# frankaging/Multimodal-Transformer

Measured on AMD Instinct MI355X. Metric: windows/sec fwd+bwd, higher is better.
Workload: dtype bf16; 1 GPU; SFT encoder stack T=500 d_model=128 heads=8 N=6 d_ff=128, 32 sequences/GPU; fwd + MSE loss + bwd (input, weight, LayerNorm grads); global_batch=32, seq_len=500, d_model=128, heads=8, layers=6, d_ff=128, parallelism=dp1, dropout=train mode, p=0.10 at the reference's four encoder sites, in-kernel generator, lengths=full

## Files before the change

include/mmt_hip.h:

```cpp
#ifndef MMT_HIP_H
#define MMT_HIP_H
#include <stddef.h>
#include <stdint.h>

#ifdef __cplusplus
extern "C" {
#endif

#define MMT_OK 0
#define MMT_EINVAL 1
#define MMT_EUNSUPPORTED 2
#define MMT_EWORKSPACE 3
#define MMT_EHIP 4

typedef void* mmt_stream_t;

int mmt_abi_version(void);
const char* mmt_last_error(void);

int mmt_profile_enable(int on);
int mmt_profile_reset(void);
int mmt_profile_num_sites(void);
const char* mmt_profile_site_name(int site);
int mmt_profile_collect(float* total_ms, int* launches);
// ... 266 lines not shown
                            void* workspace, size_t workspace_bytes, int N, int W, int D, int F, int K, mmt_stream_t stream);

size_t mmt_mse_sum_scratch_doubles(size_t n);
int mmt_mse_sum_forward(const float* pred, const float* target, float inv_denom, float* loss, float* dpred, double* scratch,
                        size_t n, mmt_stream_t stream);

int mmt_adam_step(float* const* params, const float* const* grads, float* const* exp_avg, float* const* exp_avg_sq,
                  const size_t* counts, int nchunks, float lr, float beta1, float beta2, float eps, float weight_decay,
                  int step, mmt_stream_t stream);

int mmt_ccc_forward(const float* pred, const float* target, const int32_t* lengths, double* ccc, int B, int T, mmt_stream_t stream);

int mmt_debug_dropout_mask(float p, uint64_t seed, uint32_t stream_id, uint64_t n, uint32_t attn_Tp, uint8_t* keep,
                           float* host_scale_out, mmt_stream_t stream);

int mmt_debug_poison_lds(uint32_t pattern, void* sink4, mmt_stream_t stream);

#ifdef __cplusplus
}
#endif
#endif
```

multimodal_transformer_amd/_lib.py:

```python
import ctypes
import os
import threading

import torch

_HERE = os.path.dirname(os.path.abspath(__file__))
LIB_PATH = os.environ.get("MMT_LIB_PATH") or os.path.join(_HERE, "libmmt_hip.so")

_c = ctypes
_P, _F, _I, _SZ, _U64 = _c.c_void_p, _c.c_float, _c.c_int, _c.c_size_t, _c.c_uint64

SIGNATURES = {
    "mmt_abi_version": (_I, []),
    "mmt_last_error": (_c.c_char_p, []),
    "mmt_profile_enable": (_I, [_I]),
    "mmt_profile_reset": (_I, []),
    "mmt_profile_num_sites": (_I, []),
    "mmt_profile_site_name": (_c.c_char_p, [_I]),
    "mmt_profile_collect": (_I, [_P, _P]),
    "mmt_encoder_param_count": (_SZ, [_I, _I, _I]),
    "mmt_encoder_workspace_bytes": (_SZ, [_I] * 6),
    "mmt_encoder_workspace_bytes_eval": (_SZ, [_I] * 6),
    "mmt_encoder_forward": (_I, [_P, _P, _P, _P, _P, _SZ] + [_I] * 6 + [_F, _F, _U64, _P]),
    "mmt_encoder_backward": (_I, [_P, _P, _P, _P, _P, _P, _P, _SZ] + [_I] * 6 + [_F, _F, _U64, _P]),
# ... 80 lines not shown
    "mmt_mfn_mem_scan_forward": (_I, [_P] * 9 + [_SZ] + [_I] * 4 + [_F, _U64, _P]),
    "mmt_mfn_mem_scan_forward_devseed": (_I, [_P] * 9 + [_SZ] + [_I] * 4 + [_F, _P, _P]),
    "mmt_mfn_mem_scan_backward": (_I, [_P] * 11 + [_SZ] + [_I] * 4 + [_F, _P]),
    "mmt_convpool_workspace_bytes": (_SZ, [_I] * 4),
    "mmt_convpool_forward": (_I, [_P] * 6 + [_SZ] + [_I] * 4 + [_P]),
    "mmt_convpool_backward": (_I, [_P] * 6 + [_SZ] + [_I] * 4 + [_P]),
    "mmt_convpool_k_workspace_bytes": (_SZ, [_I] * 5),
    "mmt_convpool_k_forward": (_I, [_P] * 6 + [_SZ] + [_I] * 5 + [_P]),
    "mmt_convpool_k_backward": (_I, [_P] * 6 + [_SZ] + [_I] * 5 + [_P]),
    "mmt_mse_sum_scratch_doubles": (_SZ, [_SZ]),
    "mmt_mse_sum_forward": (_I, [_P, _P, _F, _P, _P, _P, _SZ, _P]),
    "mmt_adam_step": (_I, [_P, _P, _P, _P, _P, _I, _F, _F, _F, _F, _F, _I, _P]),
    "mmt_ccc_forward": (_I, [_P, _P, _P, _P, _I, _I, _P]),
    "mmt_debug_dropout_mask": (_I, [_F, _U64, _c.c_uint32, _U64, _c.c_uint32, _P, _P, _P]),
    "mmt_debug_poison_lds": (_I, [_c.c_uint32, _P, _P]),
}


class CopySeg(ctypes.Structure):
    _fields_ = [("src", _P), ("src2", _P), ("dst", _P), ("rowscale", _P), ("rows", _I), ("cols", _I), ("src_ld", _I), ("src2_ld", _I),
                ("dst_ld", _I), ("perm", _I), ("pB", _I), ("pT", _I), ("accumulate", _I)]


_lib = None
_lock = threading.Lock()


def load():
    global _lib
    if _lib is not None:
# ... 290 lines not shown
```

multimodal_transformer_amd/csrc/api.hip:

```cpp
#include <hip/hip_runtime.h>
#include <stdarg.h>
#include <stdio.h>
#include <string.h>
#include <math.h>
#include <stdlib.h>
#include <initializer_list>
#include <mutex>
#include <type_traits>
#include <unordered_set>

#include "../../include/mmt_hip.h"
#include "common.h"
#include "attn_mask.h"
#include "rowgemm.h"
#include "attn.h"
#include "attn_bwd_pair.h"
#include "attn_probs.h"
#ifdef MMT_ABLATIONS
#include "attn_bwd_pair_diag.h"
#include "attn_fwd_diag.h"
#endif
#include "misc_kernels.h"
#include "scan_common.h"
#include "scan.h"
// ... 184 lines not shown
    D.nsplit = (D.MP + D.mchunk - 1) / D.mchunk;
    return MMT_OK;
}

static int check_drop(float dropout_p, const EncDims& D) {
    if (!(dropout_p >= 0.f && dropout_p < 1.f)) return fail(MMT_EINVAL, "dropout_p %g not in [0,1)", dropout_p);
    if (dropout_p > 0.f && D.Tp > 4096) return fail(MMT_EUNSUPPORTED, "train-mode dropout supports T <= 4096 (got %d)", D.T);
    return MMT_OK;
}

static bool use_fused_bwd(const EncDims& D) {
    static const bool allowed = getenv("MMT_NO_FUSED_ATTN_BWD") == nullptr;
    return allowed && attn_bwd_fused_ok(D.L.DKP, D.nt);
}

struct LayerWs {
    float *xout, *x1, *stats1, *stats2, *lse;
    bf16 *xn1, *xn2, *QR, *KR, *VR, *ctx, *hid;
    bf16 *dx2, *dh, *dx1, *dqkv;
    float *lnpart1, *lnpart2;
    uint16_t *maskQ, *maskK;
};
struct EncWs {
    uint64_t* seedword;
    bf16* wprep; float* bprep; float* statsf;
    LayerWs lw[MAX_LAYERS];
    float *dxa, *dxb, *delta, *lnpartf;
    bf16 *dOR;
    float *sWqkv, *sbqkv, *sWo, *sbo, *sW1, *sb1, *sW2, *sb2;
    size_t slab_stride;
// ... 116 lines not shown
static bool prep_shape_at(int shape) { return tail_fold_on() && shape == 128; }
static RowGemmParams rg_zero() { RowGemmParams p; memset(&p, 0, sizeof(p)); p.mask_scale = 1.0f; return p; }

static DropCfg no_drop() { return make_drop(0.f, 0, 0); }
#define MMT_ATTN_DROP_BITS 12
static DropCfg stream_drop(float p, uint64_t seed, uint32_t stream, bool devseed, int bits = 16, uint32_t first = 0) {
    DropCfg c = make_drop(p, seed, stream, bits);
    if (devseed) { c.s0 = stream - first; c.s1 = 0; }
    return c;
}
static int launch_seed_advance(uint64_t* state, uint64_t* block, uint32_t first, int n, hipStream_t st) {
    if (n + 1 > MMT_SEED_BLOCK_WORDS) return fail(MMT_EUNSUPPORTED, "%d dropout streams do not fit the seed block", n);
    return launch("seed_advance_kernel", seed_advance_kernel, dim3(1), dim3(128), 0, st, state, block, first, n);
}

static int fill_mask_gen(MaskGenParams& P, uint16_t* mq, uint16_t* mk, const EncDims& D, int nlayers, float p, uint64_t seed,
                         const uint64_t* seedword = nullptr) {
    if (nlayers > 16) return fail(MMT_EUNSUPPORTED, "mask generator: %d layers > 16", nlayers);
    memset(&P, 0, sizeof(P));
    P.lq = mq; P.lk = mk; P.nbh = D.B * D.h; P.nt = D.nt; P.nlayers = nlayers;
    P.layer_words = attn_mask_layer_words(P.nbh, P.nt);
    P.seedword = seedword;
    for (int l = 0; l < nlayers; ++l) { const DropCfg c = stream_drop(p, seed, 4 * l + 0, seedword != nullptr, MMT_ATTN_DROP_BITS); P.thr16 = c.thr16; P.s0[l] = c.s0; P.s1[l] = c.s1; }
    return MMT_OK;
}
static int launch_mask_gen(uint16_t* mq, uint16_t* mk, const EncDims& D, int nlayers, float p, uint64_t seed, hipStream_t st) {
    MaskGenParams P;
    int rc;
    if ((rc = fill_mask_gen(P, mq, mk, D, nlayers, p, seed))) return rc;
    const size_t blocks = (size_t)P.nbh * P.nt * P.nt;
    ProfScope prof(S_MASK_GEN, st);
    return launch("attn_mask_gen_kernel", attn_mask_gen_kernel, dim3((unsigned)((blocks + 255) / 256), nlayers), dim3(256), 0, st, P);
}

class AttnSel {
    AttnSel(AttnMode m, const int32_t* kl, int sp = 0) : mode(m), key_lengths(kl), span(sp) {}
public:
    AttnMode mode; const int32_t* key_lengths; int span;
    static AttnSel plain() { return AttnSel(ATTN_PLAIN, nullptr); }
    static AttnSel causal() { return AttnSel(ATTN_CAUSAL, nullptr); }
    static AttnSel band(int span) { return AttnSel(ATTN_BAND, nullptr, span); }
    static AttnSel keys(const int32_t* key_lengths) { return AttnSel(ATTN_KEYS, key_lengths); }
};
template <typename KP, typename KK, typename KB, typename... A>
static int launch_attn_form(const AttnSel& sel, const char* plain_name, KP* plain, const char* keys_name, KK* keys, const char* causal_name, KP* causal,
                            const char* band_name, KB* band, dim3 grid, hipStream_t st, const A&... args) {
    if (sel.mode == ATTN_KEYS) return launch(keys_name, keys, grid, dim3(MMT_THREADS), 0, st, args..., sel.key_lengths);
    if (sel.mode == ATTN_BAND) return launch(band_name, band, grid, dim3(MMT_THREADS), 0, st, args..., sel.span);
    const bool c = sel.mode == ATTN_CAUSAL;
    return launch(c ? causal_name : plain_name, c ? causal : plain, grid, dim3(MMT_THREADS), 0, st, args...);
}

static int launch_attn_fwd(int DKP, const bf16* QR, const bf16* KR, const bf16* VR, bf16* ctx, float* lse,
                           const EncDims& D, hipStream_t st, const AttnSel& sel, DropCfg drop = no_drop(), const uint16_t* maskQ = nullptr) {
    dim3 grid(attn_grid((D.nt + 3) / 4, D.B * D.h));
    if (drop.thr16 && !maskQ) return fail(MMT_EINVAL, "attention dropout without a mask buffer");
    ProfScope prof(S_ATTN_FWD, st);
#ifdef MMT_ABLATIONS
    static const bool stamp_fwd = getenv("MMT_ABL") && atoi(getenv("MMT_ABL")) == 6;
    if (stamp_fwd && sel.mode == ATTN_PLAIN && DKP == 16 && drop.thr16)
        return launch("attn_fwd_stamped_kernel", attn_fwd_stamped_kernel<16, true>, grid, dim3(MMT_THREADS), 0, st, QR, KR, VR, ctx, lse,
                      D.h, D.T, D.nt, D.B * D.h, D.L.HDP, maskQ, drop.scale, 0);
#endif
    return with_dkp(DKP, drop.thr16 != 0, [&](auto dkp, auto dr) {
        int rc = MMT_OK;
        for (int fb = 0; fb < (CT(dkp) + 31) / 32 && !rc; ++fb)
            rc = launch_attn_form(sel, "attn_fwd_kernel", attn_fwd_kernel<CT(dkp), CT(dr)>, "attn_fwd_keys_kernel", attn_fwd_keys_kernel<CT(dkp), CT(dr)>,
                                  "attn_fwd_causal_kernel", attn_fwd_causal_kernel<CT(dkp), CT(dr)>,
                                  "attn_fwd_band_kernel", attn_fwd_band_kernel<CT(dkp), CT(dr)>, grid, st,
                                  QR, KR, VR, ctx, lse, D.h, D.T, D.nt, D.B * D.h, D.L.HDP, maskQ, drop.scale, fb);
        return rc;
    });
}

static int launch_attn_bwd(int DKP, const bf16* QR, const bf16* KR, const bf16* VR,
                           const bf16* dOR, const float* lse, const float* delta, const float* rowmask,
                           bf16* dqkv, const EncDims& D, hipStream_t st, const AttnSel& sel, DropCfg drop = no_drop(),
                           const uint16_t* maskQ = nullptr, const uint16_t* maskK = nullptr) {
// ... 82 lines not shown
    if (!pointers_ok || !workspace) return fail(MMT_EINVAL, "null pointer argument");
    if ((rc = check_drop(dropout_p, C.D))) return rc;
    carve_encoder(C.W, C.D, workspace, dropout_p > 0.f);
    if ((rc = check_workspace(workspace_bytes, C.W.bytes))) return rc;
    C.st = static_cast<hipStream_t>(stream);
    C.dropout_p = dropout_p; C.seed = seed;
    C.devseed = devseed && dropout_p > 0.f;
    C.seedword = C.devseed ? C.W.seedword : nullptr;
    return MMT_OK;
}
static MaskRide layer_mask_ride(const MaskGenParams& MG, const EncWs& W, int layer, int waves, int chain_wgs) {
    MaskRide ride; memset(&ride, 0, sizeof(ride));
    ride.chain_wgs = chain_wgs;
    if (!waves) return ride;
    MaskGenLayer& g = ride.g;
    g.lq = W.lw[layer].maskQ; g.lk = W.lw[layer].maskK; g.nbh = MG.nbh; g.nt = MG.nt;
    g.thr16 = MG.thr16; g.s0 = MG.s0[layer]; g.s1 = MG.s1[layer]; g.seedword = MG.seedword;
    const size_t blocks = (size_t)g.nbh * g.nt * g.nt, per_wg = (size_t)64 * waves;
    ride.gen_waves = waves; ride.gen_wgs = (int)((blocks + per_wg - 1) / per_wg);
    return ride;
}

static int encoder_forward_impl(const float* x, const float* mask, const float* params, float* y,
                                void* workspace, size_t workspace_bytes,
                                int B, int T, int d, int h, int f, int n_layers, float eps,
                                float dropout_p, uint64_t seed, uint64_t* seed_state, mmt_stream_t stream, const AttnSel& sel) {
    EncCall C;
    C.sel = sel;
    int rc = encoder_begin(C, x && mask && params && y, workspace, workspace_bytes, B, T, d, h, f, n_layers, dropout_p, seed, seed_state != nullptr, stream);
    if (rc) return rc;
    ALIGNED16("mmt_encoder_forward", PA(x), PA(params), PA(y));
    const EncDims& D = C.D; const EncWs& W = C.W; const LayerLayout& L = D.L;
    hipStream_t st = C.st;
    const bool devseed = C.devseed;
    const uint64_t* seedword = C.seedword;

    const int shape = chain_shape(d, f, h, L);
    static const bool fuse_next_qkv = getenv("MMT_NO_CHAIN4") == nullptr;
    const int ride_waves = (dropout_p > 0.f && fuse_next_qkv)
        ? mask_ride_waves(shape, layer_geom(CHAIN_FWD, L).lds) : 0;
    const int head_waves = (dropout_p > 0.f && fuse_next_qkv && D.N > 0 && (D.N == 1 || ride_waves))
        ? mask_ride_waves(shape, layer_geom(STAGE_LN1_QKV, L).lds, MMT_HEAD_RIDE_WAVES) : 0;
    const int nstreams = 4 * D.N + 4;
    if (devseed && !head_waves && (rc = launch_seed_advance(seed_state, W.seedword, 0, nstreams, st))) return rc;
    MaskGenParams MG;
    if (D.N > 0 && dropout_p > 0.f && (rc = fill_mask_gen(MG, W.lw[0].maskQ, W.lw[0].maskK, D, D.N, dropout_p, seed, seedword))) return rc;
    if (D.N > 0 && dropout_p > 0.f && !head_waves) {
        MaskGenParams P = MG;
        if (ride_waves) P.nlayers = 1;
        const size_t blocks = (size_t)P.nbh * P.nt * P.nt;
        const int gen_blocks = (int)((blocks + 255) / 256), prep_blocks = std::min(grid_for(L.pstride() + L.qstride()), 64);
        ProfScope prof(S_MASK_GEN, st);
        LAUNCH(encoder_prep_maskgen_kernel, dim3((unsigned)(gen_blocks + prep_blocks), D.N), dim3(256), 0, st,
                           params, W.wprep, W.bprep, L, gen_blocks, P);
    } else if (D.N > 0) {
        if (devseed && nstreams + 1 > MMT_SEED_BLOCK_WORDS) return fail(MMT_EUNSUPPORTED, "%d dropout streams do not fit the seed block", nstreams);
        ProfScope prof(S_PREP, st);
        if (prep_shape_at(shape)) {
            const int prep_blocks = PrepShape<128>::blocks();
            if (devseed) LAUNCH(encoder_prep_shape_seed_kernel<128>, dim3(prep_blocks + 1, D.N), dim3(256), 0, st,
                               params, W.wprep, W.bprep, L, seed_state, W.seedword, nstreams);
// ... 440 lines not shown
}

static int sdpa_forward_impl(const float* q, const float* k, const float* v, const float* mask, float* ctx,
                             void* workspace, size_t workspace_bytes, int B, int T, int d, int h,
                             float dropout_p, uint64_t seed, mmt_stream_t stream, const AttnSel& sel) {
    SdpaCall C;
    int rc = sdpa_begin(C, q && k && v && ctx, workspace, workspace_bytes, B, T, d, h, dropout_p, stream);
    if (rc) return rc;
    const EncDims& D = C.D; const SdpaWs& W = C.W; const LayerLayout& L = D.L;
    hipStream_t st = C.st;
    const int g = grid_for((size_t)D.M * h);
    const float qs = LOG2E / sqrtf((float)L.dk);
    LAUNCH(pack_frag_kernel, dim3(g), dim3(256), 0, st, q, W.QR, mask, qs, 1, nullptr, 0, nullptr, D.M, T, D.Tp, h, L.dk, L.DKP, d);
    LAUNCH(pack_frag_kernel, dim3(g), dim3(256), 0, st, k, W.KR, nullptr, 1.f, 0, nullptr, 0, nullptr, D.M, T, D.Tp, h, L.dk, L.DKP, d);
    LAUNCH(pack_frag_kernel, dim3(g), dim3(256), 0, st, v, W.VR, nullptr, 1.f, 0, nullptr, 0, nullptr, D.M, T, D.Tp, h, L.dk, L.DKP, d);
    if (dropout_p > 0.f && (rc = launch_mask_gen(W.maskQ, W.maskK, D, 1, dropout_p, seed, st))) return rc;
    if ((rc = launch_attn_fwd(L.DKP, W.QR, W.KR, W.VR, W.ctx, W.lse, D, st, sel, make_drop(dropout_p, seed, 0, MMT_ATTN_DROP_BITS), W.maskQ))) return rc;
    LAUNCH(unpad_heads_kernel, dim3(grid_for((size_t)D.M * d)), dim3(256), 0, st, W.ctx, L.HDP, 0, ctx, D.M, h, L.dk, L.DKP, d);
    return MMT_OK;
}
extern "C" int mmt_sdpa_forward(const float* q, const float* k, const float* v, const float* mask, float* ctx,
                                void* workspace, size_t workspace_bytes, int B, int T, int d, int h,
                                float dropout_p, uint64_t seed, mmt_stream_t stream) {
    return sdpa_forward_impl(q, k, v, mask, ctx, workspace, workspace_bytes, B, T, d, h, dropout_p, seed, stream, AttnSel::plain());
}
extern "C" int mmt_sdpa_forward_keys(const float* q, const float* k, const float* v, const float* mask, float* ctx,
                                     void* workspace, size_t workspace_bytes, int B, int T, int d, int h,
                                     float dropout_p, uint64_t seed, mmt_stream_t stream, const int32_t* key_lengths) {
    if (!key_lengths) return fail(MMT_EINVAL, "null key_lengths");
    return sdpa_forward_impl(q, k, v, mask, ctx, workspace, workspace_bytes, B, T, d, h, dropout_p, seed, stream, AttnSel::keys(key_lengths));
}
// ... 1215 lines not shown

extern "C" int mmt_ccc_forward(const float* pred, const float* target, const int32_t* lengths, double* ccc, int B, int T, mmt_stream_t stream) {
    if (!pred || !target || !lengths || !ccc) return fail(MMT_EINVAL, "null pointer argument");
    if (B <= 0 || T <= 0) return fail(MMT_EINVAL, "bad shape B=%d T=%d", B, T);
    LAUNCH(ccc_kernel, dim3(B), dim3(256), 0, static_cast<hipStream_t>(stream), pred, target, lengths, ccc, T);
    return MMT_OK;
}

extern "C" int mmt_debug_poison_lds(uint32_t pattern, void* sink4, mmt_stream_t stream) {
    if (!sink4) return fail(MMT_EINVAL, "null pointer argument");
    LAUNCH(poison_lds_kernel, dim3(2048), dim3(1024), 160 * 1024, static_cast<hipStream_t>(stream), pattern, 160 * 256, static_cast<uint32_t*>(sink4));
    LAUNCH(poison_vgpr_kernel, dim3(8192), dim3(256), 0, static_cast<hipStream_t>(stream), pattern, static_cast<uint32_t*>(sink4));
    return MMT_OK;
}

extern "C" int mmt_debug_dropout_mask(float p, uint64_t seed, uint32_t stream_id, uint64_t n, uint32_t attn_Tp, uint8_t* keep,
                                      float* scale_out, mmt_stream_t stream) {
    if (!keep) return fail(MMT_EINVAL, "null pointer argument");
    const DropCfg c = make_drop(p, seed, stream_id, attn_Tp ? MMT_ATTN_DROP_BITS : 16);
    if (scale_out) *scale_out = c.scale;
    if (attn_Tp) {
        if (attn_Tp % 32 || n % ((uint64_t)attn_Tp * attn_Tp)) return fail(MMT_EINVAL, "attention mask: n must be a multiple of Tp*Tp, Tp of 32");
        const int nt = (int)(attn_Tp / 32), nbh = (int)(n / ((uint64_t)attn_Tp * attn_Tp));
        const size_t blocks = (size_t)nbh * nt * nt;
        LAUNCH(attn_mask_expand_kernel, dim3((unsigned)((blocks + 63) / 64)), dim3(64), 0, static_cast<hipStream_t>(stream), c, nbh, nt, keep);
        return MMT_OK;
    }
    LAUNCH(dropout_mask_kernel, dim3(grid_for(n)), dim3(256), 0, static_cast<hipStream_t>(stream), c, n, keep);
    return MMT_OK;
}
// ... 1 lines not shown
```

multimodal_transformer_amd/csrc/attn.h:

```cpp
#pragma once
#include <type_traits>
#include "common.h"
#include "attn_mask.h"

template <int NSEG, int MAXL = 3>
struct TileStager {
    const bf16* src[MAXL]; int stride[MAXL]; bool on[MAXL]; int dst[MAXL];
    bf16x8 reg[MAXL];
    __device__ __forceinline__ void init(const bf16* const* base, const int* pieces, const int* strides, const int* lds0, const int* pad, int tid) {
#pragma unroll
        for (int l = 0; l < MAXL; ++l) {
            const int p = tid + MMT_THREADS * l;
            int acc = 0; on[l] = false; src[l] = base[0]; stride[l] = 0; dst[l] = 0;
#pragma unroll
            for (int sg = 0; sg < NSEG; ++sg) {
                if (!on[l] && p >= acc && p < acc + pieces[sg]) {
                    on[l] = true; src[l] = base[sg] + (size_t)(p - acc) * 8; stride[l] = strides[sg];
                    dst[l] = (lds0[sg] + (p - acc) + ((p - acc) >> 5) * pad[sg]) * 8;
                }
                acc += pieces[sg];
            }
        }
    }
    __device__ __forceinline__ void load(int tile) {
// ... 44 lines not shown
    const int L = blockIdx.x, grp = L / (8 * nx), rem = L - grp * 8 * nx;
    AttnBlock a;
    a.bx = rem >> 3;
    a.bh = grp * 8 + (rem & 7);
    a.valid = a.bh < nbh;
    return a;
}
__host__ inline int attn_grid(int nx, int nbh) { return nx * 8 * ((nbh + 7) / 8); }
__device__ __forceinline__ AttnBlock attn_block_causal(int nx, int nbh) {
    AttnBlock a = attn_block(nx, nbh);
    const int grp = blockIdx.x / (8 * nx);
    a.bx = (a.bx + ((grp * nx) >> 5)) % nx;
    return a;
}

template <int DKP, bool DROP, int MODE>
__device__ __forceinline__ void attn_fwd_body(
        const bf16* __restrict__ Qr, const bf16* __restrict__ Kr, const bf16* __restrict__ Vr,
        bf16* __restrict__ ctx, float* __restrict__ lse,
        int h, int T, int nt, int nbh, int ldc, const uint16_t* __restrict__ maskQ, float drop_scale, int fb,
        const int* __restrict__ key_lengths, int span) {
    constexpr bool KEYS = MODE == ATTN_KEYS, CAUSAL = MODE == ATTN_CAUSAL, BAND = MODE == ATTN_BAND;
    constexpr int KS = DKP / 16;
    constexpr int DKB = DKP < 32 ? DKP : 32;
    constexpr bool ONES = (DKP == 16) && !DROP;
    constexpr int PK = DKP * 4, PV = DKB * 4, PVL = (DKB / 8) * MMT_TR_OCT;
    __shared__ __attribute__((aligned(16))) bf16 stage[2][(PK + PVL) * 8];
    __shared__ __attribute__((aligned(16))) bf16 zeros[256];
    const int lane = threadIdx.x & 63, wave = __builtin_amdgcn_readfirstlane(threadIdx.x >> 6);
    const int r = lane & 31, hh = lane >> 5;
    const AttnBlock ab = CAUSAL ? attn_block_causal((nt + 3) >> 2, nbh) : attn_block((nt + 3) >> 2, nbh);
    if (!ab.valid) return;
    const int qt = ab.bx * 4 + wave;
    const bool live = qt < nt;
    const int qtc = live ? qt : nt - 1;
    const int bh = ab.bh, b = bh / h, head = bh - b * h;
    const int Tp = nt * 32;
    const int Tk = KEYS ? attn_key_len(key_lengths, b, T) : T;
    const int nk = KEYS ? (Tk + 31) >> 5 : (CAUSAL || BAND) ? min(nt, ab.bx * 4 + 4) : nt;
    const int sp = BAND ? min(span, T) : 0;
    const int kw0 = BAND ? band_lo_tile(ab.bx * 4, sp) : 0, klo = BAND ? band_lo_tile(qtc, sp) : 0;
    const int kfirst = BAND ? nk - 1 : 0;
    const int qrel = BAND ? min(qtc * 32 + r, T - 1) : 0;
    const bf16* Qb = Qr + (size_t)bh * fragR_elems(Tp, DKP);
    const bf16* Kb = Kr + (size_t)bh * fragR_elems(Tp, DKP);
    const bf16* Vb = Vr + (size_t)bh * fragR_elems(Tp, DKP) + (size_t)fb * 4 * 256;
    const uint16_t* mrow = maskQ + ((size_t)bh * nt + qtc) * nt * 64 + lane;
    uint32_t mw = DROP ? mrow[BAND ? (size_t)qtc * 64 : 0] : 0u;

    TileStager<2, (PK + PV + MMT_THREADS - 1) / MMT_THREADS> stg;
    {
        const bf16* base[2] = {Kb, Vb};
        const int pieces[2] = {PK, PV}, strides[2] = {32 * DKP, 32 * DKP}, lds0[2] = {0, PK}, pad[2] = {0, MMT_TR_OCT - 32};
        stg.init(base, pieces, strides, lds0, pad, threadIdx.x);
    }
    stg.load(kfirst);
    zeros[threadIdx.x] = (bf16)0.f;
    const int g1 = (lane >> 4) & 1, tq = (lane >> 2) & 3, tpp = lane & 3;
    const int voff = ((2 * g1 + (tpp >> 1)) * MMT_TR_OCT + 4 * hh + tq) * 8 + 4 * (tpp & 1);
    const bool vpad = DKB < 32 && g1;
    bf16x8 qf[KS];
#pragma unroll
    for (int s = 0; s < KS; ++s)
// ... 8 lines not shown
#pragma unroll
    for (int i = 0; i < 16; ++i) o[i] = 0.f;
    float mrun = 0.f, lrun = 0.f;
    f32x16 mneg;
#pragma unroll
    for (int i = 0; i < 16; ++i) mneg[i] = 0.f;

    auto body = [&](auto tile_tag, int kt) {
        constexpr bool TAIL = (int)decltype(tile_tag)::value == 1, DIAG = (int)decltype(tile_tag)::value == 2;
        constexpr bool EDGE = (int)decltype(tile_tag)::value == 3;
        const bool more = BAND ? kt > kw0 : CAUSAL ? kt + 1 < nk : !TAIL;
        const int knext = BAND ? kt - 1 : kt + 1;
        progress_prio(BAND ? qt - kt : kt, BAND ? qt - klo + 1 : nk);
        const uint32_t tw = mw;
        if (BAND) { if (DROP && kt > klo) mw = mrow[(size_t)(kt - 1) * 64]; }
        else if (DROP && !TAIL && !DIAG) mw = mrow[(size_t)(kt + 1) * 64];
        if (more) stg.load(knext);
        const bf16* sk = stage[kt & 1];
        const bf16* sv = vpad ? zeros : sk + PK * 8 + voff;
        f32x16 s;
        if constexpr (KS == 1) {
            const bf16x8 kf = *reinterpret_cast<const bf16x8*>(sk + (hh * 32 + r) * 8);
            asm volatile("v_mfma_f32_32x32x16_bf16 %0, %1, %2, %3\n\ts_nop 11" : "=&v"(s) : "v"(kf), "v"(qf[0]), "v"(mneg));
        } else {
            s = mfma32(*reinterpret_cast<const bf16x8*>(sk + (hh * 32 + r) * 8), qf[0], mneg);
#pragma unroll
            for (int ss = 1; ss < KS; ++ss)
                s = mfma32(*reinterpret_cast<const bf16x8*>(sk + ((2 * ss + hh) * 32 + r) * 8), qf[ss], s);
        }
        if (TAIL) {
#pragma unroll
            for (int i = 0; i < 16; ++i) s[i] = (kt * 32 + acc32_row(i, hh) < Tk) ? s[i] : -INFINITY;
        }
        if (DIAG) {
#pragma unroll
            for (int i = 0; i < 16; ++i) s[i] = (acc32_row(i, hh) <= r && kt * 32 + acc32_row(i, hh) < T) ? s[i] : -INFINITY;
        }
// ... 13 lines not shown
            mrun += dlt;
            lrun *= alpha;
#pragma unroll
            for (int i = 0; i < 16; ++i) { o[i] *= alpha; s[i] -= dlt; }
            fill16(mneg, -mrun);
        }
#pragma unroll
        for (int i = 0; i < 16; ++i) s[i] = fast_exp2(s[i]);
        if (!ONES) {
            float a = s[0];
#pragma unroll
            for (int i = 1; i < 16; ++i) a += s[i];
            lrun += a;
        }
        if (DROP) {
            static_for<0, 16>([&](auto ic) { constexpr int i = decltype(ic)::value; s[i] = keep_and<i>(s[i], tw); });
        }
#pragma unroll
        for (int s2 = 0; s2 < 2; ++s2) {
            bf16x8 va = tr_frag2(sv + 128 * s2, sv + 128 * s2 + 64);
            if (ONES && r == DKP) va = ones;
            o = mfma32(va, pack8(s, s2), o);
        }
        if (more) stg.store(stage[knext & 1]);
        __syncthreads();
    };
    if constexpr (CAUSAL) {
        for (int kt = 0; kt < (live ? qt : 0); ++kt) body(TileFull{}, kt);
        if (live) body(TileDiag{}, qt);
        __builtin_amdgcn_s_setprio(0);
        for (int kt = live ? qt + 1 : 0; kt < nk; ++kt) {
// ... 29 lines not shown
        for (int g = 0; g < DKB / 8; ++g) {
            bf16x4 v;
#pragma unroll
            for (int i = 0; i < 4; ++i) v[i] = (bf16)(o[4 * g + i] * inv);
            const int e0 = 32 * fb + 8 * g + 4 * hh;
            *reinterpret_cast<bf16x4*>(ctx + m * ldc + head * DKP + e0) = v;
        }
    }
}
template <int DKP, bool DROP>
__global__ __launch_bounds__(MMT_THREADS, 2) void attn_fwd_kernel(
        const bf16* __restrict__ Qr, const bf16* __restrict__ Kr, const bf16* __restrict__ Vr,
        bf16* __restrict__ ctx, float* __restrict__ lse,
        int h, int T, int nt, int nbh, int ldc, const uint16_t* __restrict__ maskQ, float drop_scale, int fb) {
    attn_fwd_body<DKP, DROP, ATTN_PLAIN>(Qr, Kr, Vr, ctx, lse, h, T, nt, nbh, ldc, maskQ, drop_scale, fb, nullptr, 0);
}
template <int DKP, bool DROP>
__global__ __launch_bounds__(MMT_THREADS, 2) void attn_fwd_keys_kernel(
        const bf16* __restrict__ Qr, const bf16* __restrict__ Kr, const bf16* __restrict__ Vr,
        bf16* __restrict__ ctx, float* __restrict__ lse,
        int h, int T, int nt, int nbh, int ldc, const uint16_t* __restrict__ maskQ, float drop_scale, int fb,
        const int* __restrict__ key_lengths) {
    attn_fwd_body<DKP, DROP, ATTN_KEYS>(Qr, Kr, Vr, ctx, lse, h, T, nt, nbh, ldc, maskQ, drop_scale, fb, key_lengths, 0);
}
template <int DKP, bool DROP>
__global__ __launch_bounds__(MMT_THREADS, 2) void attn_fwd_causal_kernel(
        const bf16* __restrict__ Qr, const bf16* __restrict__ Kr, const bf16* __restrict__ Vr,
        bf16* __restrict__ ctx, float* __restrict__ lse,
        int h, int T, int nt, int nbh, int ldc, const uint16_t* __restrict__ maskQ, float drop_scale, int fb) {
    attn_fwd_body<DKP, DROP, ATTN_CAUSAL>(Qr, Kr, Vr, ctx, lse, h, T, nt, nbh, ldc, maskQ, drop_scale, fb, nullptr, 0);
// ... 435 lines not shown
```

multimodal_transformer_amd/csrc/attn_mask.h:

```cpp
#pragma once
#include "common.h"

#define MMT_MASK_BLOCK_WORDS 32

template <int CHAINS = 32>
__device__ __forceinline__ void attn_keep_block(const DropCfg& dc, uint32_t blk, uint32_t (&W)[32]) {
    static_assert(CHAINS > 0 && 32 % CHAINS == 0, "the keys of a block are drawn in equal groups");
    const uint32_t thr = dc.thr16;
    const int b0 = thr ? __builtin_ctz(thr) : 16;
    const uint32_t x0 = drop_lin(dc.s0, blk * 512u) + (uint32_t)b0 * MMT_DROP_C1;
#pragma unroll
    for (int k0 = 0; k0 < 32; k0 += CHAINS) {
        uint32_t D[CHAINS];
#pragma unroll
        for (int i = 0; i < CHAINS; ++i) D[i] = 0;
        uint32_t x = x0;
#pragma unroll 1
        for (int b = b0; b < 16; ++b) {
            if ((thr >> b) & 1u) {
#pragma unroll
                for (int i = 0; i < CHAINS; ++i) D[i] |= drop_fin(x + (uint32_t)(16 * (k0 + i)) * MMT_DROP_C1, dc.s1);
            } else {
#pragma unroll
                for (int i = 0; i < CHAINS; ++i) D[i] &= drop_fin(x + (uint32_t)(16 * (k0 + i)) * MMT_DROP_C1, dc.s1);
// ... 18 lines not shown
            A[k] ^= t << j;
        }
    }
}

__device__ __forceinline__ uint32_t lane_word(uint32_t x, int hh) {
    uint32_t y = (x >> (4 * hh)) & 0x0F0F0F0Fu;
    y = (y | (y >> 4)) & 0x00FF00FFu;
    return (y | (y >> 8)) & 0x0000FFFFu;
}

struct MaskGenParams {
    uint16_t* lq; uint16_t* lk;
    size_t layer_words;
    int nbh, nt, nlayers;
    uint32_t thr16;
    uint32_t s0[16], s1[16];
    const uint64_t* seedword;
};
struct MaskGenLayer {
    uint16_t* lq; uint16_t* lk;
    int nbh, nt;
    uint32_t thr16, s0, s1;
    const uint64_t* seedword;
};
__device__ __forceinline__ MaskGenLayer mask_gen_layer(const MaskGenParams& P, int layer) {
    MaskGenLayer G;
    G.lq = P.lq + (size_t)layer * P.layer_words; G.lk = P.lk + (size_t)layer * P.layer_words;
    G.nbh = P.nbh; G.nt = P.nt; G.thr16 = P.thr16; G.s0 = P.s0[layer]; G.s1 = P.s1[layer]; G.seedword = P.seedword;
    return G;
}

#define MMT_MASK_LDS_ROW 72
__device__ __forceinline__ void park_lane_block(uint16_t* row, const uint32_t (&rows)[32]) {
#pragma unroll
    for (int c = 0; c < 8; ++c) {
        u32x4_t v;
#pragma unroll
        for (int e = 0; e < 4; ++e) {
            const int l0 = 8 * (c & 3) + 2 * e, hh = c >> 2;
            v[e] = lane_word(rows[l0], hh) | (lane_word(rows[l0 + 1], hh) << 16);
        }
        *reinterpret_cast<u32x4_t*>(row + 8 * c) = v;
    }
}

#define MMT_MASK_PATCH_WORDS (64 * MMT_MASK_LDS_ROW)
#define MMT_MASK_GEN_WAVES 4
template <int CHAINS = 32>
__device__ __forceinline__ void attn_mask_gen_block(const MaskGenLayer& P, uint16_t* patch, size_t first, int gen_waves) {
    const int lane = threadIdx.x & 63, wave = __builtin_amdgcn_readfirstlane(threadIdx.x >> 6);
    if (wave >= gen_waves) return;
    patch += wave * MMT_MASK_PATCH_WORDS;
    const size_t g0 = first + wave * 64;
    const size_t per_bh = (size_t)P.nt * P.nt, total = (size_t)P.nbh * per_bh;
    if (g0 >= total) return;
// ... 11 lines not shown
    const uint16_t* from;
    auto flush_from = [&] { int l = lane; asm volatile("" : "+v"(l)); return patch + (l >> 3) * MMT_MASK_LDS_ROW + 8 * (l & 7); };
    park_lane_block(mine, W);
    from = flush_from();
    {
        size_t gb = g0 + (lane >> 3);
        int bb = __shfl(bh, lane >> 3), qb = __shfl(qt, lane >> 3), kb = __shfl(kt, lane >> 3);
#pragma unroll
        for (int i = 0; i < 8; ++i) {
            const u32x4_t v = *reinterpret_cast<const u32x4_t*>(from + 8 * i * MMT_MASK_LDS_ROW);
            if (gb < total) *reinterpret_cast<u32x4_t*>(P.lk + ((size_t)bb * per_bh + (size_t)kb * P.nt + qb) * 64 + 8 * fp) = v;
            gb += 8; kb += 8;
            while (kb >= P.nt) { kb -= P.nt; if (++qb == P.nt) { qb = 0; ++bb; } }
        }
    }
    transpose32(W);
    park_lane_block(mine, W);
    from = flush_from();
    {
        uint16_t* const lq = P.lq + g0 * 64;
#pragma unroll
        for (int i = 0; i < 8; ++i) {
            const u32x4_t v = *reinterpret_cast<const u32x4_t*>(from + 8 * i * MMT_MASK_LDS_ROW);
            if (g0 + 8 * i + (lane >> 3) < total) *reinterpret_cast<u32x4_t*>(lq + (size_t)i * 512 + lane * 8) = v;
        }
    }
}

__global__ __launch_bounds__(256, 4) void attn_mask_gen_kernel(const MaskGenParams P) {
    __shared__ __attribute__((aligned(16))) uint16_t patch[MMT_MASK_GEN_WAVES * MMT_MASK_PATCH_WORDS];
    attn_mask_gen_block(mask_gen_layer(P, blockIdx.y), patch, (size_t)blockIdx.x * (64 * MMT_MASK_GEN_WAVES), MMT_MASK_GEN_WAVES);
}

__host__ inline size_t attn_mask_layer_words(int nbh, int nt) { return (size_t)nbh * nt * nt * 64; }

template <int I> struct IdxC { static constexpr int value = I; };
template <int B, int E, class F> __device__ __forceinline__ void static_for(F&& f) {
    if constexpr (B < E) { f(IdxC<B>{}); static_for<B + 1, E>(f); }
}
template <int I> __device__ __forceinline__ uint32_t keep_bits(uint32_t w) {
    uint32_t m;
    asm("v_bfe_i32 %0, %1, %2, 1" : "=v"(m) : "v"(w), "n"(I));
    return m;
}
template <int I> __device__ __forceinline__ float keep_and(float v, uint32_t w) {
    return __builtin_bit_cast(float, __builtin_bit_cast(uint32_t, v) & keep_bits<I>(w));
}

__global__ void attn_mask_expand_kernel(DropCfg base, int nbh, int nt, uint8_t* __restrict__ keep) {
    const size_t g = (size_t)blockIdx.x * blockDim.x + threadIdx.x;
    const size_t per_bh = (size_t)nt * nt;
    const int bh = (int)(g / per_bh);
    if (bh >= nbh) return;
    const int rem = (int)(g - (size_t)bh * per_bh), qt = rem / nt, kt = rem - qt * nt;
    const DropCfg dc = drop_substream(base, (uint32_t)bh);
    uint32_t W[32];
    attn_keep_block(dc, (uint32_t)(qt * nt + kt), W);
    const size_t Tp = (size_t)nt * 32;
#pragma unroll
    for (int key = 0; key < 32; ++key)
#pragma unroll 1
// ... 4 lines not shown
```

multimodal_transformer_amd/functional.py:

```python
import ctypes
import math

import torch

from . import _lib


def _f32c(t):
    return t.detach().contiguous().float() if t is not None else None


def _f32c16(t):
    t = _f32c(t)
    return t.clone() if t is not None and t.data_ptr() % 16 else t


def _seed_arg(seed):
    if isinstance(seed, (list, tuple)):
        return [_seed_arg(v) for v in seed]
    return seed if isinstance(seed, _lib.DeviceSeed) else int(seed)


def _seed_pair(seed):
    return (0, seed.state) if isinstance(seed, _lib.DeviceSeed) else (int(seed), None)
# ... 1713 lines not shown

def lstm_stream_step_slots(x_t, mask_t, state, positions, in_dim, embed_dim, h_dim, n_layers, attn_len, limit=None, advance=True):
    return _lstm_step("lstm_stream_step_slots", x_t, mask_t, state, (in_dim, embed_dim, h_dim, n_layers, attn_len), positions=positions,
                      limit=limit, advance=advance)


def check_device_errors():
    _lib.ERRORS.check()


def poison_lds(device, pattern=0x7FC00000):
    sink = torch.zeros(1, dtype=torch.int32, device=device)
    _lib.launch("mmt_debug_poison_lds", int(pattern), sink)


def dropout_mask(p, seed, stream_id, n, device, attn_Tp=0):
    keep = torch.empty(n, dtype=torch.uint8, device=device)
    sc = ctypes.c_float(0.0)
    _lib.launch("mmt_debug_dropout_mask", float(p), int(seed), int(stream_id), int(n), int(attn_Tp), keep,
                ctypes.cast(ctypes.pointer(sc), ctypes.c_void_p))
    return keep.bool(), float(sc.value)
```

Baseline: 21.30 million windows/s.

## Store attention dropout masks as per-register lane bitmasks loaded via scalar loads

```diff
diff --git a/include/mmt_hip.h b/include/mmt_hip.h
--- a/include/mmt_hip.h
+++ b/include/mmt_hip.h
@@ -304,6 +304,9 @@
 int mmt_debug_dropout_mask(float p, uint64_t seed, uint32_t stream_id, uint64_t n, uint32_t attn_Tp, uint8_t* keep,
                            float* host_scale_out, mmt_stream_t stream);
 
+int mmt_debug_attn_mask_words(float p, uint64_t seed, uint32_t stream_id, int nbh, int nt, int lanes,
+                              uint16_t* lq, uint16_t* lk, mmt_stream_t stream);
+
 int mmt_debug_poison_lds(uint32_t pattern, void* sink4, mmt_stream_t stream);
 
 #ifdef __cplusplus
diff --git a/multimodal_transformer_amd/_lib.py b/multimodal_transformer_amd/_lib.py
--- a/multimodal_transformer_amd/_lib.py
+++ b/multimodal_transformer_amd/_lib.py
@@ -118,6 +118,7 @@
     "mmt_ccc_forward": (_I, [_P, _P, _P, _P, _I, _I, _P]),
     "mmt_debug_dropout_mask": (_I, [_F, _U64, _c.c_uint32, _U64, _c.c_uint32, _P, _P, _P]),
     "mmt_debug_poison_lds": (_I, [_c.c_uint32, _P, _P]),
+    "mmt_debug_attn_mask_words": (_I, [_F, _U64, _c.c_uint32, _I, _I, _I, _P, _P, _P]),
 }
 
 
diff --git a/multimodal_transformer_amd/csrc/api.hip b/multimodal_transformer_amd/csrc/api.hip
--- a/multimodal_transformer_amd/csrc/api.hip
+++ b/multimodal_transformer_amd/csrc/api.hip
@@ -222,6 +222,11 @@
     return allowed && attn_bwd_fused_ok(D.L.DKP, D.nt);
 }
 
+static bool use_lane_masks(const EncDims& D, AttnMode mode) {
+    static const bool allowed = getenv("MMT_NO_LANE_MASKS") == nullptr;
+    return allowed && mode == ATTN_PLAIN && D.L.DKP == 16 && use_fused_bwd(D);
+}
+
 struct LayerWs {
     float *xout, *x1, *stats1, *stats2, *lse;
     bf16 *xn1, *xn2, *QR, *KR, *VR, *ctx, *hid;
@@ -368,20 +373,21 @@
     return launch("seed_advance_kernel", seed_advance_kernel, dim3(1), dim3(128), 0, st, state, block, first, n);
 }
 
-static int fill_mask_gen(MaskGenParams& P, uint16_t* mq, uint16_t* mk, const EncDims& D, int nlayers, float p, uint64_t seed,
+static int fill_mask_gen(MaskGenParams& P, uint16_t* mq, uint16_t* mk, const EncDims& D, int nlayers, float p, uint64_t seed, bool lanes,
                          const uint64_t* seedword = nullptr) {
     if (nlayers > 16) return fail(MMT_EUNSUPPORTED, "mask generator: %d layers > 16", nlayers);
     memset(&P, 0, sizeof(P));
     P.lq = mq; P.lk = mk; P.nbh = D.B * D.h; P.nt = D.nt; P.nlayers = nlayers;
     P.layer_words = attn_mask_layer_words(P.nbh, P.nt);
+    P.lanes = lanes;
     P.seedword = seedword;
     for (int l = 0; l < nlayers; ++l) { const DropCfg c = stream_drop(p, seed, 4 * l + 0, seedword != nullptr, MMT_ATTN_DROP_BITS); P.thr16 = c.thr16; P.s0[l] = c.s0; P.s1[l] = c.s1; }
     return MMT_OK;
 }
-static int launch_mask_gen(uint16_t* mq, uint16_t* mk, const EncDims& D, int nlayers, float p, uint64_t seed, hipStream_t st) {
+static int launch_mask_gen(uint16_t* mq, uint16_t* mk, const EncDims& D, int nlayers, float p, uint64_t seed, bool lanes, hipStream_t st) {
     MaskGenParams P;
     int rc;
-    if ((rc = fill_mask_gen(P, mq, mk, D, nlayers, p, seed))) return rc;
+    if ((rc = fill_mask_gen(P, mq, mk, D, nlayers, p, seed, lanes))) return rc;
     const size_t blocks = (size_t)P.nbh * P.nt * P.nt;
     ProfScope prof(S_MASK_GEN, st);
     return launch("attn_mask_gen_kernel", attn_mask_gen_kernel, dim3((unsigned)((blocks + 255) / 256), nlayers), dim3(256), 0, st, P);
@@ -409,13 +415,17 @@
                            const EncDims& D, hipStream_t st, const AttnSel& sel, DropCfg drop = no_drop(), const uint16_t* maskQ = nullptr) {
     dim3 grid(attn_grid((D.nt + 3) / 4, D.B * D.h));
     if (drop.thr16 && !maskQ) return fail(MMT_EINVAL, "attention dropout without a mask buffer");
+    const bool lanes = drop.thr16 && use_lane_masks(D, sel.mode);
     ProfScope prof(S_ATTN_FWD, st);
 #ifdef MMT_ABLATIONS
     static const bool stamp_fwd = getenv("MMT_ABL") && atoi(getenv("MMT_ABL")) == 6;
     if (stamp_fwd && sel.mode == ATTN_PLAIN && DKP == 16 && drop.thr16)
-        return launch("attn_fwd_stamped_kernel", attn_fwd_stamped_kernel<16, true>, grid, dim3(MMT_THREADS), 0, st, QR, KR, VR, ctx, lse,
+        return launch("attn_fwd_stamped_kernel", lanes ? attn_fwd_lanes16_stamped_kernel<true> : attn_fwd_stamped_kernel<16, true>, grid, dim3(MMT_THREADS), 0, st, QR, KR, VR, ctx, lse,
                       D.h, D.T, D.nt, D.B * D.h, D.L.HDP, maskQ, drop.scale, 0);
 #endif
+    if (lanes)
+        return launch("attn_fwd_kernel", attn_fwd_lanes16_kernel<true>, grid, dim3(MMT_THREADS), 0, st,
+                      QR, KR, VR, ctx, lse, D.h, D.T, D.nt, D.B * D.h, D.L.HDP, maskQ, drop.scale, 0);
     return with_dkp(DKP, drop.thr16 != 0, [&](auto dkp, auto dr) {
         int rc = MMT_OK;
         for (int fb = 0; fb < (CT(dkp) + 31) / 32 && !rc; ++fb)
@@ -528,7 +538,7 @@
     ride.chain_wgs = chain_wgs;
     if (!waves) return ride;
     MaskGenLayer& g = ride.g;
-    g.lq = W.lw[layer].maskQ; g.lk = W.lw[layer].maskK; g.nbh = MG.nbh; g.nt = MG.nt;
+    g.lq = W.lw[layer].maskQ; g.lk = W.lw[layer].maskK; g.nbh = MG.nbh; g.nt = MG.nt; g.lanes = MG.lanes;
     g.thr16 = MG.thr16; g.s0 = MG.s0[layer]; g.s1 = MG.s1[layer]; g.seedword = MG.seedword;
     const size_t blocks = (size_t)g.nbh * g.nt * g.nt, per_wg = (size_t)64 * waves;
     ride.gen_waves = waves; ride.gen_wgs = (int)((blocks + per_wg - 1) / per_wg);
@@ -558,7 +568,7 @@
     const int nstreams = 4 * D.N + 4;
     if (devseed && !head_waves && (rc = launch_seed_advance(seed_state, W.seedword, 0, nstreams, st))) return rc;
     MaskGenParams MG;
-    if (D.N > 0 && dropout_p > 0.f && (rc = fill_mask_gen(MG, W.lw[0].maskQ, W.lw[0].maskK, D, D.N, dropout_p, seed, seedword))) return rc;
+    if (D.N > 0 && dropout_p > 0.f && (rc = fill_mask_gen(MG, W.lw[0].maskQ, W.lw[0].maskK, D, D.N, dropout_p, seed, use_lane_masks(D, C.sel.mode), seedword))) return rc;
     if (D.N > 0 && dropout_p > 0.f && !head_waves) {
         MaskGenParams P = MG;
         if (ride_waves) P.nlayers = 1;
@@ -1029,7 +1039,7 @@
     LAUNCH(pack_frag_kernel, dim3(g), dim3(256), 0, st, q, W.QR, mask, qs, 1, nullptr, 0, nullptr, D.M, T, D.Tp, h, L.dk, L.DKP, d);
     LAUNCH(pack_frag_kernel, dim3(g), dim3(256), 0, st, k, W.KR, nullptr, 1.f, 0, nullptr, 0, nullptr, D.M, T, D.Tp, h, L.dk, L.DKP, d);
     LAUNCH(pack_frag_kernel, dim3(g), dim3(256), 0, st, v, W.VR, nullptr, 1.f, 0, nullptr, 0, nullptr, D.M, T, D.Tp, h, L.dk, L.DKP, d);
-    if (dropout_p > 0.f && (rc = launch_mask_gen(W.maskQ, W.maskK, D, 1, dropout_p, seed, st))) return rc;
+    if (dropout_p > 0.f && (rc = launch_mask_gen(W.maskQ, W.maskK, D, 1, dropout_p, seed, use_lane_masks(D, sel.mode), st))) return rc;
     if ((rc = launch_attn_fwd(L.DKP, W.QR, W.KR, W.VR, W.ctx, W.lse, D, st, sel, make_drop(dropout_p, seed, 0, MMT_ATTN_DROP_BITS), W.maskQ))) return rc;
     LAUNCH(unpad_heads_kernel, dim3(grid_for((size_t)D.M * d)), dim3(256), 0, st, W.ctx, L.HDP, 0, ctx, D.M, h, L.dk, L.DKP, d);
     return MMT_OK;
@@ -2275,6 +2285,20 @@
     return MMT_OK;
 }
 
+extern "C" int mmt_debug_attn_mask_words(float p, uint64_t seed, uint32_t stream_id, int nbh, int nt, int lanes,
+                                         uint16_t* lq, uint16_t* lk, mmt_stream_t stream) {
+    if (!lq || !lk) return fail(MMT_EINVAL, "null pointer argument");
+    if (nbh < 1 || nt < 1 || nt > 128) return fail(MMT_EINVAL, "attention mask words: nbh >= 1, 1 <= nt <= 128");
+    const DropCfg c = make_drop(p, seed, stream_id, MMT_ATTN_DROP_BITS);
+    MaskGenParams P;
+    memset(&P, 0, sizeof(P));
+    P.lq = lq; P.lk = lk; P.nbh = nbh; P.nt = nt; P.nlayers = 1; P.layer_words = attn_mask_layer_words(nbh, nt);
+    P.lanes = lanes != 0; P.thr16 = c.thr16; P.s0[0] = c.s0; P.s1[0] = c.s1;
+    const size_t blocks = (size_t)nbh * nt * nt;
+    return launch("attn_mask_gen_kernel", attn_mask_gen_kernel, dim3((unsigned)((blocks + 255) / 256), 1), dim3(256), 0,
+                  static_cast<hipStream_t>(stream), P);
+}
+
 extern "C" int mmt_debug_dropout_mask(float p, uint64_t seed, uint32_t stream_id, uint64_t n, uint32_t attn_Tp, uint8_t* keep,
                                       float* scale_out, mmt_stream_t stream) {
     if (!keep) return fail(MMT_EINVAL, "null pointer argument");
diff --git a/multimodal_transformer_amd/csrc/attn.h b/multimodal_transformer_amd/csrc/attn.h
--- a/multimodal_transformer_amd/csrc/attn.h
+++ b/multimodal_transformer_amd/csrc/attn.h
@@ -82,7 +82,7 @@
     return a;
 }
 
-template <int DKP, bool DROP, int MODE>
+template <int DKP, bool DROP, int MODE, bool LANES = false>
 __device__ __forceinline__ void attn_fwd_body(
         const bf16* __restrict__ Qr, const bf16* __restrict__ Kr, const bf16* __restrict__ Vr,
         bf16* __restrict__ ctx, float* __restrict__ lse,
@@ -92,6 +92,7 @@
     constexpr int KS = DKP / 16;
     constexpr int DKB = DKP < 32 ? DKP : 32;
     constexpr bool ONES = (DKP == 16) && !DROP;
+    static_assert(!LANES || (DROP && DKP == 16 && MODE == ATTN_PLAIN), "lane masks: the plain d_k = 16 train kernel only");
     constexpr int PK = DKP * 4, PV = DKB * 4, PVL = (DKB / 8) * MMT_TR_OCT;
     __shared__ __attribute__((aligned(16))) bf16 stage[2][(PK + PVL) * 8];
     __shared__ __attribute__((aligned(16))) bf16 zeros[256];
@@ -114,7 +115,8 @@
     const bf16* Kb = Kr + (size_t)bh * fragR_elems(Tp, DKP);
     const bf16* Vb = Vr + (size_t)bh * fragR_elems(Tp, DKP) + (size_t)fb * 4 * 256;
     const uint16_t* mrow = maskQ + ((size_t)bh * nt + qtc) * nt * 64 + lane;
-    uint32_t mw = DROP ? mrow[BAND ? (size_t)qtc * 64 : 0] : 0u;
+    uint32_t mw = (DROP && !LANES) ? mrow[BAND ? (size_t)qtc * 64 : 0] : 0u;
+    const uint32_t mblk0 = LANES ? __builtin_amdgcn_readfirstlane((uint32_t)((bh * nt + qtc) * nt)) : 0u;
 
     TileStager<2, (PK + PV + MMT_THREADS - 1) / MMT_THREADS> stg;
     {
@@ -153,13 +155,20 @@
         progress_prio(BAND ? qt - kt : kt, BAND ? qt - klo + 1 : nk);
         const uint32_t tw = mw;
         if (BAND) { if (DROP && kt > klo) mw = mrow[(size_t)(kt - 1) * 64]; }
-        else if (DROP && !TAIL && !DIAG) mw = mrow[(size_t)(kt + 1) * 64];
+        else if (DROP && !LANES && !TAIL && !DIAG) mw = mrow[(size_t)(kt + 1) * 64];
         if (more) stg.load(knext);
         const bf16* sk = stage[kt & 1];
         const bf16* sv = vpad ? zeros : sk + PK * 8 + voff;
         f32x16 s;
+        LaneMasks lm;
         if constexpr (KS == 1) {
             const bf16x8 kf = *reinterpret_cast<const bf16x8*>(sk + (hh * 32 + r) * 8);
+            if constexpr (LANES) {
+                uint32_t blk = mblk0 + (uint32_t)kt;
+                asm volatile("" : "+s"(blk) : "v"(kf));
+                lm = load_lane_masks(maskQ + (size_t)blk * 64);
+                __builtin_amdgcn_sched_barrier(0);
+            }
             asm volatile("v_mfma_f32_32x32x16_bf16 %0, %1, %2, %3\n\ts_nop 11" : "=&v"(s) : "v"(kf), "v"(qf[0]), "v"(mneg));
         } else {
             s = mfma32(*reinterpret_cast<const bf16x8*>(sk + (hh * 32 + r) * 8), qf[0], mneg);
@@ -203,7 +212,10 @@
             lrun += a;
         }
         if (DROP) {
-            static_for<0, 16>([&](auto ic) { constexpr int i = decltype(ic)::value; s[i] = keep_and<i>(s[i], tw); });
+            if constexpr (LANES) {
+#pragma unroll
+                for (int i = 0; i < 8; ++i) { s[i] = keep_lanes(s[i], lm.lo[i]); s[8 + i] = keep_lanes(s[8 + i], lm.hi[i]); }
+            } else static_for<0, 16>([&](auto ic) { constexpr int i = decltype(ic)::value; s[i] = keep_and<i>(s[i], tw); });
         }
 #pragma unroll
         for (int s2 = 0; s2 < 2; ++s2) {
@@ -263,6 +275,13 @@
         bf16* __restrict__ ctx, float* __restrict__ lse,
         int h, int T, int nt, int nbh, int ldc, const uint16_t* __restrict__ maskQ, float drop_scale, int fb) {
     attn_fwd_body<DKP, DROP, ATTN_PLAIN>(Qr, Kr, Vr, ctx, lse, h, T, nt, nbh, ldc, maskQ, drop_scale, fb, nullptr, 0);
+}
+template <bool DROP>
+__global__ __launch_bounds__(MMT_THREADS, 2) void attn_fwd_lanes16_kernel(
+        const bf16* __restrict__ Qr, const bf16* __restrict__ Kr, const bf16* __restrict__ Vr,
+        bf16* __restrict__ ctx, float* __restrict__ lse,
+        int h, int T, int nt, int nbh, int ldc, const uint16_t* __restrict__ maskQ, float drop_scale, int fb) {
+    attn_fwd_body<16, DROP, ATTN_PLAIN, true>(Qr, Kr, Vr, ctx, lse, h, T, nt, nbh, ldc, maskQ, drop_scale, fb, nullptr, 0);
 }
 template <int DKP, bool DROP>
 __global__ __launch_bounds__(MMT_THREADS, 2) void attn_fwd_keys_kernel(
diff --git a/multimodal_transformer_amd/csrc/attn_mask.h b/multimodal_transformer_amd/csrc/attn_mask.h
--- a/multimodal_transformer_amd/csrc/attn_mask.h
+++ b/multimodal_transformer_amd/csrc/attn_mask.h
@@ -56,6 +56,7 @@
     uint16_t* lq; uint16_t* lk;
     size_t layer_words;
     int nbh, nt, nlayers;
+    int lanes;
     uint32_t thr16;
     uint32_t s0[16], s1[16];
     const uint64_t* seedword;
@@ -63,13 +64,14 @@
 struct MaskGenLayer {
     uint16_t* lq; uint16_t* lk;
     int nbh, nt;
+    int lanes;
     uint32_t thr16, s0, s1;
     const uint64_t* seedword;
 };
 __device__ __forceinline__ MaskGenLayer mask_gen_layer(const MaskGenParams& P, int layer) {
     MaskGenLayer G;
     G.lq = P.lq + (size_t)layer * P.layer_words; G.lk = P.lk + (size_t)layer * P.layer_words;
-    G.nbh = P.nbh; G.nt = P.nt; G.thr16 = P.thr16; G.s0 = P.s0[layer]; G.s1 = P.s1[layer]; G.seedword = P.seedword;
+    G.nbh = P.nbh; G.nt = P.nt; G.lanes = P.lanes; G.thr16 = P.thr16; G.s0 = P.s0[layer]; G.s1 = P.s1[layer]; G.seedword = P.seedword;
     return G;
 }
 
@@ -82,6 +84,19 @@
         for (int e = 0; e < 4; ++e) {
             const int l0 = 8 * (c & 3) + 2 * e, hh = c >> 2;
             v[e] = lane_word(rows[l0], hh) | (lane_word(rows[l0 + 1], hh) << 16);
+        }
+        *reinterpret_cast<u32x4_t*>(row + 8 * c) = v;
+    }
+}
+
+__device__ __forceinline__ void park_lane_masks(uint16_t* row, const uint32_t (&W)[32]) {
+#pragma unroll
+    for (int c = 0; c < 8; ++c) {
+        u32x4_t v;
+#pragma unroll
+        for (int e = 0; e < 4; ++e) {
+            const int i = 2 * c + (e >> 1), hh = e & 1;
+            v[e] = W[(i & 3) + 8 * (i >> 2) + 4 * hh];
         }
         *reinterpret_cast<u32x4_t*>(row + 8 * c) = v;
     }
@@ -123,8 +138,11 @@
             while (kb >= P.nt) { kb -= P.nt; if (++qb == P.nt) { qb = 0; ++bb; } }
         }
     }
-    transpose32(W);
-    park_lane_block(mine, W);
+    if (P.lanes) park_lane_masks(mine, W);
+    else {
+        transpose32(W);
+        park_lane_block(mine, W);
+    }
     from = flush_from();
     {
         uint16_t* const lq = P.lq + g0 * 64;
@@ -154,6 +172,18 @@
 }
 template <int I> __device__ __forceinline__ float keep_and(float v, uint32_t w) {
     return __builtin_bit_cast(float, __builtin_bit_cast(uint32_t, v) & keep_bits<I>(w));
+}
+__device__ __forceinline__ float keep_lanes(float v, uint64_t m) {
+    return __builtin_amdgcn_inverse_ballot_w64(m) ? v : 0.f;
+}
+typedef uint64_t u64x8_t __attribute__((ext_vector_type(8)));
+struct LaneMasks { u64x8_t lo, hi; };
+__device__ __forceinline__ LaneMasks load_lane_masks(const uint16_t* block) {
+    typedef const volatile u64x8_t __attribute__((address_space(4))) * cptr;
+    const cptr p = (cptr)(uintptr_t)block;
+    LaneMasks m;
+    m.lo = p[0]; m.hi = p[1];
+    return m;
 }
 
 __global__ void attn_mask_expand_kernel(DropCfg base, int nbh, int nt, uint8_t* __restrict__ keep) {
diff --git a/multimodal_transformer_amd/functional.py b/multimodal_transformer_amd/functional.py
--- a/multimodal_transformer_amd/functional.py
+++ b/multimodal_transformer_amd/functional.py
@@ -1751,6 +1751,13 @@
     _lib.launch("mmt_debug_poison_lds", int(pattern), sink)
 
 
+def _attn_mask_words(p, seed, stream_id, nbh, nt, device, lanes=False):
+    lq = torch.empty(nbh * nt * nt, 64, dtype=torch.int16, device=device)
+    lk = torch.empty_like(lq)
+    _lib.launch("mmt_debug_attn_mask_words", float(p), int(seed), int(stream_id), int(nbh), int(nt), int(bool(lanes)), lq, lk)
+    return lq, lk
+
+
 def dropout_mask(p, seed, stream_id, n, device, attn_Tp=0):
     keep = torch.empty(n, dtype=torch.uint8, device=device)
     sc = ctypes.c_float(0.0)
```

After: 21.52 million windows/s (median of 6 runs). +1.1%, better.
